# impromptuRong/hd_yolo

Measured on AMD Instinct MI355X. Metric: tiles/sec (640x640) fwd+bwd, higher is better.
Workload: dtype bf16; 1 GPU; metayolo yolov5s 8-class nuclei, 640x640 RGB tiles, batch 64/GPU, train step = fwd + DetLoss + bwd + all-reduce + SGD(nesterov); global_batch=64, parallelism=dp1, world_size=1, backend=none, hw_queues=4

## Files before the change

hd_yolo_amd/build.py:

```python
import os
import subprocess
import sys
from concurrent.futures import ThreadPoolExecutor

HERE = os.path.dirname(os.path.abspath(__file__))
CSRC = os.path.join(HERE, 'csrc')
OUT = os.path.join(CSRC, 'build')
LIB = os.path.join(OUT, 'libhdyolo_hip.so')
SOURCES = ['api.hip', 'conv_dispatch.hip', 'conv_igemm.hip', 'conv3x3.hip', 'conv3x3_c128.hip', 'conv3x3s2.hip', 'conv_deep.hip', 'conv_stem.hip', 'conv_wgrad.hip', 'conv_wgrad3x3.hip', 'conv_wgrad_deep.hip', 'conv_dgrad_s2.hip', 'conv1x1_bwd.hip', 'bn_act.hip', 'pool.hip', 'detect.hip', 'nms_grid.hip', 'slide.hip', 'augment.hip', 'augment_masks.hip', 'score.hip', 'paste.hip', 'mask_score.hip', 'loss.hip', 'roi.hip', 'seg.hip', 'optim.hip', 'exec.hip']
FLAGS = ['--offload-arch=gfx950', '-O3', '-fPIC', '-std=c++17', '-ffp-contract=off', '-Wall', '-Wno-unused-function',
         '-I' + CSRC, '-I' + os.path.join(os.path.dirname(HERE), 'include')]


def _newer(a, bs):
    return os.path.exists(a) and all(os.path.getmtime(a) >= os.path.getmtime(b) for b in bs)


def build(force=False, verbose=True):
    os.makedirs(OUT, exist_ok=True)
    headers = [os.path.join(CSRC, h) for h in os.listdir(CSRC) if h.endswith('.h')]
    headers.append(os.path.join(os.path.dirname(HERE), 'include', 'hdyolo.h'))
    hipcc = os.environ.get('HIPCC', '/opt/rocm/bin/hipcc')

    def compile_one(src):
        s = os.path.join(CSRC, src)
        o = os.path.join(OUT, src.replace('.hip', '.o'))
        if not force and _newer(o, [s] + headers):
            return o
        cmd = [hipcc] + FLAGS + ['-c', s, '-o', o]
        if verbose:
            print(' '.join(cmd), flush=True)
        subprocess.check_call(cmd)
        return o

    with ThreadPoolExecutor(max_workers=min(6, os.cpu_count() or 1)) as ex:
        objs = list(ex.map(compile_one, SOURCES))
    if force or not _newer(LIB, objs):
        cmd = [hipcc, '--offload-arch=gfx950', '-shared', '-fPIC', '-o', LIB] + objs
        if verbose:
            print(' '.join(cmd), flush=True)
        subprocess.check_call(cmd)
    return LIB


if __name__ == '__main__':
    print(build(force='--force' in sys.argv))
```

hd_yolo_amd/csrc/api.hip:

```cpp
#include <stdarg.h>
#include <stdio.h>
#include <stdlib.h>
#include <string.h>

#include <atomic>

#include "common.h"
#include "hdyolo_internal.h"
#include "hdyolo.h"

int hdy_pack_weight_launch(const hdy_pack_desc& d, hipStream_t st);
int hdy_pack_batch_launch(const hdy_pack_desc* table, int n, int total_blocks, hipStream_t st);

static thread_local char g_err[512] = "";

void hdy_set_error(const char* fmt, ...) {
    va_list ap;
    va_start(ap, fmt);
    vsnprintf(g_err, sizeof(g_err), fmt, ap);
    va_end(ap);
}

namespace {
struct OptDef { const char* name; int def; bool flag; };
const OptDef g_opt_def[HDY_OPT_COUNT] = {
    {"HDY_NO_CLASS_WALK", 0, true}, {"HDY_NO_CONV3X3", 0, true}, {"HDY_C3_GRID", 0, false}, {"HDY_NO_CONV3X3S2", 0, false},
    {"HDY_NO_DGRAD_S2", 0, false}, {"HDY_TILE_INTERLEAVE", 1, false}, {"HDY_NO_BIG_TILES", 0, true}, {"HDY_NO_STEM_KERNEL", 0, true},
    {"HDY_WGRAD_BLOCKS", 512, false}, {"HDY_NO_STEM_WGRAD", 0, true}, {"HDY_NO_WGRAD3X3", 0, true}, 
    {"HDY_LOSS_GRID", 2048, false}, {"HDY_NO_DEEP", 0, true}, {"HDY_NO_WGRAD_DEEP", 0, true}, {"HDY_DEEP_BN", 0, false}, {"HDY_DEEP_DEBUG", 0, false}, {"HDY_DEEP_ALL", 1, false}, {"HDY_DEEP_MIN_TILES", 160, false}, {"HDY_DEEP_WALK", 2, false}, {"HDY_NO_BN_REDUCE4", 0, true},
    {"HDY_WGRAD_TILE", 0, false}, {"HDY_SPPF_NO_KEYS", 0, true}, {"HDY_WGRAD_DEEP_KMIN", 192, false}, {"HDY_NO_CONV3X3_C128", 0, true}, {"HDY_NO_F1X1_96", 0, true},
    {"HDY_AP_CHUNK", 0, false}, {"HDY_AP_NO_PRUNE", 0, true},
};
std::atomic<int> g_opt[HDY_OPT_COUNT];
std::once_flag g_opt_once;
void opt_init() {
    std::call_once(g_opt_once, [] {
        for (int i = 0; i < HDY_OPT_COUNT; ++i) {
            const char* v = getenv(g_opt_def[i].name);
            g_opt[i].store(v ? (g_opt_def[i].flag ? 1 : atoi(v)) : g_opt_def[i].def, std::memory_order_relaxed);
        }
    });
}
int opt_index(const char* name) {
    for (int i = 0; name && i < HDY_OPT_COUNT; ++i)
        if (!strcmp(name, g_opt_def[i].name)) return i;
    return -1;
}
thread_local char g_disp_last[64] = "";
std::mutex g_disp_mu;
char g_disp_log[32768] = "";
size_t g_disp_len = 0;
thread_local char g_disp_copy[32768] = "";
}

int hdy_opt(int id) {
    opt_init();
    return g_opt[id].load(std::memory_order_relaxed);
}

void hdy_note_dispatch(const char* what) {
    snprintf(g_disp_last, sizeof(g_disp_last), "%s", what);
    const size_t n = strlen(g_disp_last);
    std::lock_guard<std::mutex> lock(g_disp_mu);
    if (g_disp_len + n + 2 < sizeof(g_disp_log)) {
        memcpy(g_disp_log + g_disp_len, g_disp_last, n);
        g_disp_log[g_disp_len + n] = ';';
        g_disp_log[g_disp_len + n + 1] = 0;
        g_disp_len += n + 1;
    }
}

namespace {

enum { KIND_FWD = 0, KIND_DGRAD = 1, KIND_STEM = 2 };

inline int velems(int dtype) { return dtype == HDY_BF16 ? 8 : 4; }
inline int bke(int dtype) { return 8 * velems(dtype); }
inline size_t esize(int dtype) { return dtype == HDY_BF16 ? 2 : 4; }

inline size_t block_elems(int rows, int kd, int dtype) {
    const int bn = hdy_conv_bn_tile(rows);
    return (size_t)round_up(rows, bn) * round_up(kd, bke(dtype));
}

}

extern "C" {

const char* hdy_last_error(void) { return g_err; }

const char* hdy_last_dispatch(void) { return g_disp_last; }

const char* hdy_dispatch_log(void) {
    std::lock_guard<std::mutex> lock(g_disp_mu);
    memcpy(g_disp_copy, g_disp_log, g_disp_len + 1);
    return g_disp_copy;
}

void hdy_dispatch_log_reset(void) {
    std::lock_guard<std::mutex> lock(g_disp_mu);
    g_disp_log[0] = 0;
    g_disp_len = 0;
    g_disp_last[0] = 0;
}

int hdy_set_option(const char* name, int value) {
    const int i = opt_index(name);
    HDY_ARG(i >= 0, "set_option: unknown option %s", name ? name : "(null)");
    opt_init();
    return g_opt[i].exchange(value, std::memory_order_relaxed);
}
// ... 101 lines not shown
```

hd_yolo_amd/csrc/common.h:

```cpp
#pragma once
#include <hip/hip_runtime.h>
#include <stdint.h>
#include <stddef.h>

#include <mutex>

#define HDY_OK 0
#define HDY_EINVAL (-1)
#define HDY_EUNSUPPORTED (-2)

enum { HDY_F32 = 0, HDY_BF16 = 1 };

void hdy_set_error(const char* fmt, ...);

enum HdyOption {
    HDY_OPT_NO_CLASS_WALK,
    HDY_OPT_NO_CONV3X3,
    HDY_OPT_C3_GRID,
    HDY_OPT_NO_CONV3X3S2,
    HDY_OPT_NO_DGRAD_S2,
    HDY_OPT_TILE_INTERLEAVE,
    HDY_OPT_NO_BIG_TILES,
    HDY_OPT_NO_STEM_KERNEL,
    HDY_OPT_WGRAD_BLOCKS,
    HDY_OPT_NO_STEM_WGRAD,
    HDY_OPT_NO_WGRAD3X3,
    HDY_OPT_LOSS_GRID,
    HDY_OPT_NO_DEEP,
    HDY_OPT_NO_WGRAD_DEEP,
    HDY_OPT_DEEP_BN,
    HDY_OPT_DEEP_DEBUG,
    HDY_OPT_DEEP_ALL,
    HDY_OPT_DEEP_MIN_TILES,
    HDY_OPT_DEEP_WALK,
    HDY_OPT_NO_BN_REDUCE4,
    HDY_OPT_WGRAD_TILE,
    HDY_OPT_SPPF_NO_KEYS,
    HDY_OPT_WGRAD_DEEP_KMIN,
    HDY_OPT_NO_CONV3X3_C128,
    HDY_OPT_NO_F1X1_96,
    HDY_OPT_AP_CHUNK,
    HDY_OPT_AP_NO_PRUNE,
    HDY_OPT_COUNT
};
int hdy_opt(int id);

void hdy_note_dispatch(const char* what);

#define HDY_ARG(cond, ...)                 \
    do {                                   \
        if (!(cond)) {                     \
            hdy_set_error(__VA_ARGS__);    \
            return HDY_EINVAL;             \
        }                                  \
    } while (0)

#define HDY_LAUNCH_CHECK(what)                                                       \
    do {                                                                             \
        hipError_t e__ = hipGetLastError();                                          \
        if (e__ != hipSuccess) {                                                     \
            hdy_set_error("%s: launch failed: %s", what, hipGetErrorString(e__));    \
            return (int)e__;                                                         \
        }                                                                            \
    } while (0)

typedef __bf16 bf16_t;
typedef int i32x4 __attribute__((ext_vector_type(4)));
typedef float f32x4 __attribute__((ext_vector_type(4)));
typedef __bf16 bf16x8 __attribute__((ext_vector_type(8)));
typedef __bf16 bf16x4 __attribute__((ext_vector_type(4)));

#if defined(__HIPCC__)
__device__ __forceinline__ float row_sum16(float v) {
#ifdef HDY_ROW_SUM_SHFL
    for (int m = 1; m < 16; m <<= 1) v += __shfl_xor(v, m);
    return v;
#endif
    v += __builtin_bit_cast(float, __builtin_amdgcn_update_dpp(0, __builtin_bit_cast(int, v), 0x128, 0xF, 0xF, true));
    v += __builtin_bit_cast(float, __builtin_amdgcn_update_dpp(0, __builtin_bit_cast(int, v), 0x124, 0xF, 0xF, true));
    v += __builtin_bit_cast(float, __builtin_amdgcn_update_dpp(0, __builtin_bit_cast(int, v), 0x122, 0xF, 0xF, true));
    v += __builtin_bit_cast(float, __builtin_amdgcn_update_dpp(0, __builtin_bit_cast(int, v), 0x121, 0xF, 0xF, true));
    return v;
}
#endif

struct PerDeviceOnce {
    std::once_flag flag[16];
    template <typename F> void run(F&& fn) {
        int dev = 0;
        (void)hipGetDevice(&dev);
        std::call_once(flag[dev & 15], fn);
    }
};

static inline int cdiv(long long a, long long b) { return (int)((a + b - 1) / b); }
static inline int round_up(int a, int b) { return (a + b - 1) / b * b; }

#ifdef __HIPCC__
union V16 {
    i32x4 i;
    f32x4 f;
    bf16x8 h;
};

__device__ __forceinline__ float silu_f(float u) { return u / (1.0f + __expf(-u)); }
__device__ __forceinline__ float sigmoid_f(float u) { return 1.0f / (1.0f + __expf(-u)); }

template <typename T> __device__ __forceinline__ float to_f32(T v);
template <> __device__ __forceinline__ float to_f32<float>(float v) { return v; }
// ... 97 lines not shown
```

hd_yolo_amd/csrc/conv_dispatch.hip:

```cpp
#include "common.h"
#include "hdyolo_internal.h"
#include "hdyolo.h"

static inline int bke(int dtype) { return dtype == HDY_BF16 ? 64 : 32; }

static ConvPlan conv_fwd_plan(const ConvShape& s, int first = CONV_STEM) {
    ConvPlan p = {};
    if (first <= CONV_STEM && hdy_conv_stem_plan(s, &p)) return p;
    if (first <= CONV_3X3_C64 && hdy_conv3x3_c64_plan(s, &p)) return p;
    if (first <= CONV_3X3_C128 && hdy_conv3x3_c128_plan(s, &p)) return p;
    if (first <= CONV_3X3S2 && hdy_conv3x3s2_plan(s, &p)) return p;
    if (first <= CONV_DGRAD_S2 && hdy_dgrad3x3s2_plan(s, &p)) return p;
    if (first <= CONV_DEEP && hdy_conv_deep_plan(s, &p)) return p;
    hdy_conv_igemm_plan(s, &p);
    return p;
}

extern "C" int hdy_conv_stat_slabs(int N, int H, int W, int C, int K, int R, int S, int stride, int pad, int dtype) {
    const int stem = C == 3 && R == 6 && S == 6 && stride == 2 && pad == 2;
    return conv_fwd_plan(conv_shape(N, H, W, C, K, R, S, stride, pad, dtype, stem, 1)).slabs;
}

static int launch_planned(const ConvArgs& a, const ConvPlan& p, int dtype, int out_f32, hipStream_t st) {
    switch (p.family) {
// ... 118 lines not shown
                c.c_nkb[i] = Kdp / bke(dtype); c.c_oh[i] = ca; c.c_ow[i] = cb; c.c_w[i] = (long long)off;
                off += (size_t)rows_total * Kdp;
            }
        c.w = w_packed_dgrad;
        c.dh0 = c.c_dh[0]; c.dw0 = c.c_dw[0]; c.TH = c.c_TH[0]; c.TW = c.c_TW[0]; c.oh_off = c.ow_off = 0;
        c.Kdp = c.c_nkb[0] * bke(dtype);
        return hdy_conv_launch(c, dgrad_shape(N, H, W, C, K, R, S, stride, pad, dtype), 0, (hipStream_t)stream);
    }
    for (int ca = 0; ca < 2; ++ca)
        for (int cb = 0; cb < 2; ++cb) {
            const Axis ah = class_axis(R, pad, ca), aw = class_axis(S, pad, cb);
            ConvArgs c = a;
            c.Ho = (H - ca + 1) / 2; c.Wo = (W - cb + 1) / 2;
            c.oh_mul = c.ow_mul = 2; c.oh_off = ca; c.ow_off = cb; c.dense_out = 0;
            if (!ah.taps || !aw.taps) {
                HDY_ARG(false, "conv_dgrad: kernel %dx%d pad %d leaves a parity class without taps (unsupported)", R, S, pad);
            }
            if (c.Ho <= 0 || c.Wo <= 0) continue;
            c.dh0 = ah.d0; c.dw0 = aw.d0; c.TH = ah.taps; c.TW = aw.taps;
            c.Kdp = round_up(ah.taps * aw.taps * K, bke(dtype));
            c.w = (const char*)w_packed_dgrad + off * (dtype == HDY_BF16 ? 2 : 4);
            off += (size_t)rows_total * c.Kdp;
            const ConvShape s = {N, Ho, Wo, c.Ho, c.Wo, K, C, ah.taps, aw.taps, 1, -1, 0, dtype, 0, 0, 1};
            const int rc = hdy_conv_launch(c, s, 0, (hipStream_t)stream);
            if (rc) return rc;
        }
    return HDY_OK;
}

extern "C" {

int hdy_conv_fwd(const void* x, int ldx, const void* w_packed, const float* scale, const float* shift, const void* res, int ldr, void* y,
                 int ldy, float* stats, int stat_slabs, int N, int H, int W, int C, int K, int R, int S, int stride, int pad, int act, int accumulate,
                 int dtype, int out_f32, int stem, void* stream) {
    HDY_ARG(!stats || stat_slabs > 0, "conv_fwd: stats given with stat_slabs = %d", stat_slabs);
    HDY_ARG(stride >= 1 && R >= 1 && S >= 1 && pad >= 0, "conv_fwd: bad window");
    HDY_ARG(dtype == HDY_BF16 || dtype == HDY_F32, "conv_fwd: unknown dtype %d", dtype);
    ConvArgs a = {};
    a.x = x; a.w = w_packed; a.y = y; a.scale = scale; a.shift = shift; a.stats = stats; a.stat_cap = stat_slabs; a.res = res; a.ldr = ldr;
    HDY_ARG(!res || ldr >= K, "conv_fwd: residual pitch %d < K", ldr);
    a.N = N;
    a.Ho = conv_out_dim(H, R, stride, pad);
    a.Wo = conv_out_dim(W, S, stride, pad);
    HDY_ARG(a.Ho > 0 && a.Wo > 0, "conv_fwd: empty output");
    a.K = K; a.ldy = ldy;
    a.Hout = a.Ho; a.Wout = a.Wo; a.oh_mul = a.ow_mul = 1; a.oh_off = a.ow_off = 0; a.dense_out = 1;
    a.act = act; a.accumulate = accumulate;
    if (stem) {
        HDY_ARG(C == 3 && R == 6 && S == 6 && stride == 2 && pad == 2 && ldx == 4, "conv_fwd: stem expects C=3 k=6 s=2 p=2 on a 4-channel padded image");
        a.Hin = H + 2 * pad; a.Win = W + 2 * pad; a.C = 24; a.ldx = 4; a.span_pixels = 1;
        a.ih_mul = 2; a.iw_mul = 2; a.dh0 = 0; a.dw0 = 0; a.TH = 6; a.TW = 1;
        a.Kdp = round_up(6 * 24, bke(dtype));
    } else {
        a.Hin = H; a.Win = W; a.C = C; a.ldx = ldx;
        a.ih_mul = stride; a.iw_mul = stride; a.dh0 = -pad; a.dw0 = -pad; a.TH = R; a.TW = S;
        a.Kdp = round_up(R * S * C, bke(dtype));
    }
    return hdy_conv_launch(a, conv_shape(N, H, W, C, K, R, S, stride, pad, dtype, stem != 0, stats != nullptr), out_f32, (hipStream_t)stream);
}

int hdy_conv_dgrad(const void* dy, int lddy, const void* w_packed_dgrad, void* dx, int lddx, int N, int H, int W, int C, int K, int R,
                   int S, int stride, int pad, int accumulate, int dtype, void* stream) {
    return dgrad_impl(dy, lddy, w_packed_dgrad, dx, lddx, N, H, W, C, K, R, S, stride, pad, accumulate, dtype, nullptr, 0, stream);
}

int hdy_conv_dgrad_stats(const void* dy, int lddy, const void* w_packed_dgrad, void* dx, int lddx, int N, int H, int W, int C, int K, int R,
                         int S, int stride, int pad, int accumulate, int dtype, const hdy_stat_req* stats, int nstat, void* stream) {
    HDY_ARG(nstat >= 0 && nstat <= 2 && (nstat == 0 || stats), "conv_dgrad_stats: bad request count");
    HDY_ARG(nstat == 0 || hdy_conv_dgrad_stat_slabs(N, H, W, C, K, R, S, stride, pad, dtype) > 0, "conv_dgrad_stats: this shape cannot serve statistics");
    return dgrad_impl(dy, lddy, w_packed_dgrad, dx, lddx, N, H, W, C, K, R, S, stride, pad, accumulate, dtype, stats, nstat, stream);
}

int hdy_conv_dgrad_stat_slabs(int N, int H, int W, int C, int K, int R, int S, int stride, int pad, int dtype) {
    if (dtype != HDY_BF16 || C % 8 || hdy_conv_bn_tile(C) > 64 || (stride != 1 && stride != 2)) return 0;
    if (stride == 2 && !dgrad_class_walk(H, W, R, S, pad)) return 0;
    return conv_fwd_plan(dgrad_shape(N, H, W, C, K, R, S, stride, pad, dtype), CONV_IGEMM).grid;
}

}

static WgradPlan wgrad_plan(const WgradShape& s, int first = WGRAD_STEM) {
    WgradPlan p = {};
    if (first <= WGRAD_STEM && hdy_wgrad_stem_plan(s, &p)) return p;
    if (first <= WGRAD_3X3 && hdy_wgrad3x3_plan(s, &p)) return p;
    if (first <= WGRAD_DEEP && hdy_wgrad_deep_plan(s, &p)) return p;
    hdy_wgrad_generic_plan(s, &p);
    return p;
}

static int wgrad_launch_planned(const WgradArgs& a, const WgradPlan& p, hipStream_t st) {
    switch (p.family) {
        case WGRAD_STEM: return hdy_wgrad_stem_launch(a, p, st);
        case WGRAD_3X3: return hdy_wgrad3x3_launch(a, p, st);
        case WGRAD_DEEP: return hdy_wgrad_deep_launch(a, p, st);
        default: return hdy_wgrad_generic_launch(a, p, st);
    }
}

static WgradArgs wgrad_args(const WgradShape& s, const void* x, int ldx, const void* dy, int lddy, void* workspace) {
    WgradArgs a = {};
    a.x = x; a.dy = dy; a.partial = (float*)workspace;
    a.N = s.N; a.K = s.K; a.lddy = lddy; a.Ho = s.Ho; a.Wo = s.Wo;
    if (s.stem) {
        a.Hin = s.H + 2 * s.pad; a.Win = s.W + 2 * s.pad; a.C = 24; a.ldx = 4; a.span_pixels = 1;
        a.ih_mul = a.iw_mul = 2; a.dh0 = a.dw0 = 0; a.TH = 6; a.TW = 1;
    } else {
        a.Hin = s.H; a.Win = s.W; a.C = s.C; a.ldx = ldx;
        a.ih_mul = a.iw_mul = s.stride; a.dh0 = a.dw0 = -s.pad; a.TH = s.R; a.TW = s.S;
    }
    return a;
}

static int wgrad_run(const WgradShape& s, const WgradArgs& a, float* grad_a, int K_a, float* grad_b, int K_b, int accumulate, size_t ws_bytes, hipStream_t st) {
    const int VE = s.dtype == HDY_BF16 ? 8 : 4;
    HDY_ARG(grad_a && K_a > 0 && K_a + K_b <= a.K && K_b >= 0 && (K_b == 0) == (grad_b == nullptr), "wgrad: bad gradient split");
    HDY_ARG(a.x && a.dy && a.partial, "wgrad: null pointer");
    HDY_ARG(a.C % VE == 0 && a.K % VE == 0, "wgrad: C=%d and K=%d must be multiples of %d", a.C, a.K, VE);
    HDY_ARG(a.ldx % (a.span_pixels ? 4 : VE) == 0 && a.lddy % VE == 0 && (a.span_pixels || a.ldx >= a.C) && a.lddy >= a.K, "wgrad: bad pitches ldx=%d lddy=%d", a.ldx, a.lddy);
    HDY_ARG(((uintptr_t)a.x & 15) == 0 && ((uintptr_t)a.dy & 15) == 0, "wgrad: x/dy must be 16-byte aligned");
    HDY_ARG((long long)a.N * a.Hin * a.Win < (1LL << 31) && (long long)a.N * a.Ho * a.Wo < (1LL << 31), "wgrad: too many pixels");
    HDY_ARG(ws_bytes >= hdy_conv_wgrad_workspace_bytes(s.N, s.H, s.W, s.C, s.K, s.R, s.S, s.stride, s.pad, s.dtype, s.stem), "wgrad: workspace too small");
    WgradPlan p;
    int rc;
    for (int first = WGRAD_STEM;; first = p.family + 1) {
        p = wgrad_plan(s, first);
        rc = wgrad_launch_planned(a, p, st);
        if (rc != HDY_CONV_DECLINE) break;
    }
    if (rc) return rc;
    return hdy_wgrad_reduce(a.partial, p.splits, s.K, wgrad_cols(s), s.stem, s.C, s.R, s.S, grad_a, K_a, grad_b, K_b, accumulate, st);
}

extern "C" {

size_t hdy_conv_wgrad_workspace_bytes(int N, int H, int W, int C, int K, int R, int S, int stride, int pad, int dtype, int stem) {
    const WgradShape s = wgrad_shape(N, H, W, C, K, R, S, stride, pad, dtype, stem);
    int splits = 0;
    for (int first = WGRAD_STEM; first <= WGRAD_GENERIC;) {
        const WgradPlan p = wgrad_plan(s, first);
        if (p.splits > splits) splits = p.splits;
        first = p.family + 1;
    }
    return (size_t)splits * K * wgrad_cols(s) * sizeof(float);
}

int hdy_conv_wgrad(const void* x, int ldx, const void* dy, int lddy, int N, int H, int W, int C, int K, int R, int S, int stride, int pad,
                   float* grad_a, int K_a, float* grad_b, int K_b, int accumulate, void* workspace, size_t ws_bytes, int dtype, int stem,
                   void* stream) {
    HDY_ARG(dtype == HDY_BF16 || dtype == HDY_F32, "conv_wgrad: unknown dtype %d", dtype);
    const WgradShape s = wgrad_shape(N, H, W, C, K, R, S, stride, pad, dtype, stem != 0);
    HDY_ARG(s.Ho > 0 && s.Wo > 0, "conv_wgrad: empty dy");
    HDY_ARG(!stem || (C == 3 && R == 6 && S == 6 && stride == 2 && pad == 2 && ldx == 4), "conv_wgrad: stem expects C=3 k=6 s=2 p=2 on a 4-channel padded image");
    return wgrad_run(s, wgrad_args(s, x, ldx, dy, lddy, workspace), grad_a, K_a, grad_b, K_b, accumulate, ws_bytes, (hipStream_t)stream);
}

int hdy_conv_wgrad_stem_fused_ok(int N, int H, int W, int K) {
    WgradPlan p;
    return (K == 16 || K == 32 || K == 64) && hdy_wgrad_stem_plan(wgrad_shape(N, H, W, 3, K, 6, 6, 2, 2, HDY_BF16, 1), &p);
}

int hdy_conv_wgrad_stem_fused(const void* x, const void* dz, int lddz, const void* y, int ldy, const float* scale, const float* shift, const float* mean,
                              const float* invstd, const float* c1, const float* c2, int N, int H, int W, int K, float* grad_a, int K_a, float* grad_b,
                              int K_b, int accumulate, void* workspace, size_t ws_bytes, void* stream) {
    HDY_ARG(y, "conv_wgrad_stem_fused: null pointer");
    HDY_ARG(hdy_conv_wgrad_stem_fused_ok(N, H, W, K), "conv_wgrad_stem_fused: shape not served (K in {16, 32, 64}, output a multiple of 16 x 32)");
    const WgradShape s = wgrad_shape(N, H, W, 3, K, 6, 6, 2, 2, HDY_BF16, 1);
    WgradArgs a = wgrad_args(s, x, 4, dz, lddz, workspace);
    a.y = y; a.ldy = ldy; a.bn_scale = scale; a.bn_shift = shift; a.bn_mean = mean; a.bn_invstd = invstd; a.bn_c1 = c1; a.bn_c2 = c2;
    return wgrad_run(s, a, grad_a, K_a, grad_b, K_b, accumulate, ws_bytes, (hipStream_t)stream);
}

}
```

hd_yolo_amd/csrc/hdyolo_internal.h:

```cpp
#pragma once
#include <type_traits>

#include "common.h"

struct StatReq {
    const void* y; int ldy;
    const float *scale, *shift;
    float* slabs;
    int c0, c1, act;
    int nslabs;
};

struct ConvArgs {
    const void* x;
    const void* w;
    void* y;
    const float* scale;
    const float* shift;
    float* stats;
    int stat_cap;
    const void* res;
    int ldr;
    int N, Hin, Win, C, ldx;
    int Ho, Wo, K, ldy;
// ... 60 lines not shown

bool hdy_conv_stem_plan(const ConvShape& s, ConvPlan* p);
bool hdy_conv3x3_c64_plan(const ConvShape& s, ConvPlan* p);
bool hdy_conv3x3_c128_plan(const ConvShape& s, ConvPlan* p);
bool hdy_conv3x3s2_plan(const ConvShape& s, ConvPlan* p);
bool hdy_dgrad3x3s2_plan(const ConvShape& s, ConvPlan* p);
bool hdy_conv_deep_plan(const ConvShape& s, ConvPlan* p);
bool hdy_conv_igemm_plan(const ConvShape& s, ConvPlan* p);

enum { HDY_CONV_DECLINE = -100 };
int hdy_conv_stem_launch(const ConvArgs& a, const ConvPlan& p, int out_f32, hipStream_t st);
int hdy_conv3x3_c64_launch(const ConvArgs& a, const ConvPlan& p, int out_f32, hipStream_t st);
int hdy_conv3x3_c128_launch(const ConvArgs& a, const ConvPlan& p, int out_f32, hipStream_t st);
int hdy_conv3x3s2_launch(const ConvArgs& a, const ConvPlan& p, int out_f32, hipStream_t st);
int hdy_dgrad3x3s2_launch(const ConvArgs& a, const ConvPlan& p, int out_f32, hipStream_t st);
int hdy_conv_deep_launch(const ConvArgs& a, const ConvPlan& p, int out_f32, hipStream_t st);
int hdy_conv_igemm_launch(const ConvArgs& a, const ConvPlan& p, int dtype, int out_f32, hipStream_t st);

inline int hdy_conv_take(const ConvArgs& a, const ConvPlan& p, bool fits, const char* who) {
    if (!fits && !a.stats) return HDY_CONV_DECLINE;
    HDY_ARG(fits, "%s: statistics requested, but this call does not fit the kernel their slabs were sized for (bf16 output, 16-byte aligned x/y/res rows; "
            "ldx=%d ldy=%d)", who, a.ldx, a.ldy);
    HDY_ARG(!a.stats || a.stat_cap == p.slabs, "%s: the statistics array holds %d slabs, this launch writes %d (a kernel-selection option changed between "
            "hdy_conv_stat_slabs and the launch?)", who, a.stat_cap, p.slabs);
    return HDY_OK;
}

inline bool rows_aligned(const ConvArgs& a, bool need_w) {
    return a.ldx % 8 == 0 && a.ldy % 8 == 0 && (((uintptr_t)a.x | (uintptr_t)a.y) & 15) == 0 && (!need_w || (((uintptr_t)a.w & 15) == 0 && a.Kdp % 8 == 0)) &&
           (!a.res || (a.ldr % 8 == 0 && ((uintptr_t)a.res & 15) == 0));
}

inline int epilogue_of(const ConvArgs& a) { return a.act == 1 ? 2 : ((a.scale || a.shift) ? 1 : 0); }

template <typename F> inline void with_stats_epi(bool stats, int epi, F&& f) {
    auto with_epi = [&](auto s) {
        if (epi == 2) f(s, std::integral_constant<int, 2>{});
        else if (epi == 1) f(s, std::integral_constant<int, 1>{});
        else f(s, std::integral_constant<int, 0>{});
    };
    if (stats) with_epi(std::true_type{});
    else with_epi(std::false_type{});
}

inline int hdy_launch_status(const char* who) {
    HDY_LAUNCH_CHECK(who);
    return HDY_OK;
}

inline void hdy_magic(unsigned d, unsigned* mg, int* sh) {
    int s = 0;
    while ((1ull << s) < d) ++s;
    *mg = (unsigned)((((unsigned long long)1 << (31 + s)) + d - 1) / d);
    *sh = s;
}

struct WgradArgs {
    const void* x;
    const void* dy;
    float* partial;
    int N, Hin, Win, C, ldx;
    int Ho, Wo, K, lddy;
    int ih_mul, iw_mul, dh0, dw0, TH, TW;
    int Q, P;
    int splits, pix_per_split;
    int ktiles, qtiles;
    int span_pixels;
    const void* y; int ldy;
    const float *bn_scale, *bn_shift, *bn_mean, *bn_invstd, *bn_c1, *bn_c2;
};

struct WgradShape {
    int N, H, W;
    int Ho, Wo;
    int C, K, R, S, stride, pad, dtype;
    int stem;
};
inline WgradShape wgrad_shape(int N, int H, int W, int C, int K, int R, int S, int stride, int pad, int dtype, int stem) {
    return WgradShape{N, H, W, conv_out_dim(H, R, stride, pad), conv_out_dim(W, S, stride, pad), C, K, R, S, stride, pad, dtype, stem};
}
inline long long wgrad_pixels(const WgradShape& s) { return (long long)s.N * s.Ho * s.Wo; }
inline int wgrad_cols(const WgradShape& s) { return s.R * s.S * (s.stem ? 4 : s.C); }

enum WgradFamily { WGRAD_STEM, WGRAD_3X3, WGRAD_DEEP, WGRAD_GENERIC };

struct WgradPlan {
    int family;
    int variant;
    int grid;
    int splits;
    int pix_per_split;
    int ktiles, qtiles;
    int TOH, TOW, tiles_h, tiles_w;
};

bool hdy_wgrad_stem_plan(const WgradShape& s, WgradPlan* p);
bool hdy_wgrad3x3_plan(const WgradShape& s, WgradPlan* p);
bool hdy_wgrad_deep_plan(const WgradShape& s, WgradPlan* p);
bool hdy_wgrad_generic_plan(const WgradShape& s, WgradPlan* p);

int hdy_wgrad_stem_launch(const WgradArgs& a, const WgradPlan& p, hipStream_t st);
int hdy_wgrad3x3_launch(const WgradArgs& a, const WgradPlan& p, hipStream_t st);
int hdy_wgrad_deep_launch(const WgradArgs& a, const WgradPlan& p, hipStream_t st);
int hdy_wgrad_generic_launch(const WgradArgs& a, const WgradPlan& p, hipStream_t st);
int hdy_wgrad_reduce(const float* partial, int splits, int K, int Q, int mode, int C, int R, int S, float* grad_a, int K_a, float* grad_b, int K_b,
                     int accumulate, hipStream_t st);
```

Measured before the change: 5510 tiles/s.

## Add dedicated 3x3 stride-2 weight-gradient kernel with parity-plane patch tiling

Adds a new wgrad kernel for 3x3 stride-2 pad-1 bf16 convolutions (C=32/K=64 or C,K multiples of 64 with K<192). It stages dy tiles and a parity-split input patch into double-buffered LDS via global_load_lds, and reuses each patch load across three kernel-column taps with MFMA accumulation. The goal is to replace the generic wgrad path for the downsampling convs in the yolov5s backbone. It uses about 140KB of LDS and 768-thread blocks, and it is limited to at most 2 K×C blocks unless an option allows more.

```diff
diff --git a/hd_yolo_amd/build.py b/hd_yolo_amd/build.py
--- a/hd_yolo_amd/build.py
+++ b/hd_yolo_amd/build.py
@@ -7,7 +7,7 @@
 CSRC = os.path.join(HERE, 'csrc')
 OUT = os.path.join(CSRC, 'build')
 LIB = os.path.join(OUT, 'libhdyolo_hip.so')
-SOURCES = ['api.hip', 'conv_dispatch.hip', 'conv_igemm.hip', 'conv3x3.hip', 'conv3x3_c128.hip', 'conv3x3s2.hip', 'conv_deep.hip', 'conv_stem.hip', 'conv_wgrad.hip', 'conv_wgrad3x3.hip', 'conv_wgrad_deep.hip', 'conv_dgrad_s2.hip', 'conv1x1_bwd.hip', 'bn_act.hip', 'pool.hip', 'detect.hip', 'nms_grid.hip', 'slide.hip', 'augment.hip', 'augment_masks.hip', 'score.hip', 'paste.hip', 'mask_score.hip', 'loss.hip', 'roi.hip', 'seg.hip', 'optim.hip', 'exec.hip']
+SOURCES = ['api.hip', 'conv_dispatch.hip', 'conv_igemm.hip', 'conv3x3.hip', 'conv3x3_c128.hip', 'conv3x3s2.hip', 'conv_deep.hip', 'conv_stem.hip', 'conv_wgrad.hip', 'conv_wgrad3x3.hip', 'conv_wgrad3x3s2.hip', 'conv_wgrad_deep.hip', 'conv_dgrad_s2.hip', 'conv1x1_bwd.hip', 'bn_act.hip', 'pool.hip', 'detect.hip', 'nms_grid.hip', 'slide.hip', 'augment.hip', 'augment_masks.hip', 'score.hip', 'paste.hip', 'mask_score.hip', 'loss.hip', 'roi.hip', 'seg.hip', 'optim.hip', 'exec.hip']
 FLAGS = ['--offload-arch=gfx950', '-O3', '-fPIC', '-std=c++17', '-ffp-contract=off', '-Wall', '-Wno-unused-function',
          '-I' + CSRC, '-I' + os.path.join(os.path.dirname(HERE), 'include')]
 
diff --git a/hd_yolo_amd/csrc/api.hip b/hd_yolo_amd/csrc/api.hip
--- a/hd_yolo_amd/csrc/api.hip
+++ b/hd_yolo_amd/csrc/api.hip
@@ -26,7 +26,7 @@
 const OptDef g_opt_def[HDY_OPT_COUNT] = {
     {"HDY_NO_CLASS_WALK", 0, true}, {"HDY_NO_CONV3X3", 0, true}, {"HDY_C3_GRID", 0, false}, {"HDY_NO_CONV3X3S2", 0, false},
     {"HDY_NO_DGRAD_S2", 0, false}, {"HDY_TILE_INTERLEAVE", 1, false}, {"HDY_NO_BIG_TILES", 0, true}, {"HDY_NO_STEM_KERNEL", 0, true},
-    {"HDY_WGRAD_BLOCKS", 512, false}, {"HDY_NO_STEM_WGRAD", 0, true}, {"HDY_NO_WGRAD3X3", 0, true}, 
+    {"HDY_WGRAD_BLOCKS", 512, false}, {"HDY_NO_STEM_WGRAD", 0, true}, {"HDY_NO_WGRAD3X3", 0, true}, {"HDY_NO_WGRAD3X3S2", 0, false},
     {"HDY_LOSS_GRID", 2048, false}, {"HDY_NO_DEEP", 0, true}, {"HDY_NO_WGRAD_DEEP", 0, true}, {"HDY_DEEP_BN", 0, false}, {"HDY_DEEP_DEBUG", 0, false}, {"HDY_DEEP_ALL", 1, false}, {"HDY_DEEP_MIN_TILES", 160, false}, {"HDY_DEEP_WALK", 2, false}, {"HDY_NO_BN_REDUCE4", 0, true},
     {"HDY_WGRAD_TILE", 0, false}, {"HDY_SPPF_NO_KEYS", 0, true}, {"HDY_WGRAD_DEEP_KMIN", 192, false}, {"HDY_NO_CONV3X3_C128", 0, true}, {"HDY_NO_F1X1_96", 0, true},
     {"HDY_AP_CHUNK", 0, false}, {"HDY_AP_NO_PRUNE", 0, true},
diff --git a/hd_yolo_amd/csrc/common.h b/hd_yolo_amd/csrc/common.h
--- a/hd_yolo_amd/csrc/common.h
+++ b/hd_yolo_amd/csrc/common.h
@@ -25,6 +25,7 @@
     HDY_OPT_WGRAD_BLOCKS,
     HDY_OPT_NO_STEM_WGRAD,
     HDY_OPT_NO_WGRAD3X3,
+    HDY_OPT_NO_WGRAD3X3S2,
     HDY_OPT_LOSS_GRID,
     HDY_OPT_NO_DEEP,
     HDY_OPT_NO_WGRAD_DEEP,
diff --git a/hd_yolo_amd/csrc/conv_dispatch.hip b/hd_yolo_amd/csrc/conv_dispatch.hip
--- a/hd_yolo_amd/csrc/conv_dispatch.hip
+++ b/hd_yolo_amd/csrc/conv_dispatch.hip
@@ -224,6 +224,7 @@
 static WgradPlan wgrad_plan(const WgradShape& s, int first = WGRAD_STEM) {
     WgradPlan p = {};
     if (first <= WGRAD_STEM && hdy_wgrad_stem_plan(s, &p)) return p;
+    if (first <= WGRAD_3X3S2 && hdy_wgrad3x3s2_plan(s, &p)) return p;
     if (first <= WGRAD_3X3 && hdy_wgrad3x3_plan(s, &p)) return p;
     if (first <= WGRAD_DEEP && hdy_wgrad_deep_plan(s, &p)) return p;
     hdy_wgrad_generic_plan(s, &p);
@@ -233,6 +234,7 @@
 static int wgrad_launch_planned(const WgradArgs& a, const WgradPlan& p, hipStream_t st) {
     switch (p.family) {
         case WGRAD_STEM: return hdy_wgrad_stem_launch(a, p, st);
+        case WGRAD_3X3S2: return hdy_wgrad3x3s2_launch(a, p, st);
         case WGRAD_3X3: return hdy_wgrad3x3_launch(a, p, st);
         case WGRAD_DEEP: return hdy_wgrad_deep_launch(a, p, st);
         default: return hdy_wgrad_generic_launch(a, p, st);
diff --git a/hd_yolo_amd/csrc/conv_wgrad3x3s2.hip b/hd_yolo_amd/csrc/conv_wgrad3x3s2.hip
--- /dev/null
+++ b/hd_yolo_amd/csrc/conv_wgrad3x3s2.hip
@@ -0,0 +1,305 @@
+#include <stdlib.h>
+
+#include "common.h"
+#include "hdyolo_internal.h"
+#include "hdyolo.h"
+
+__device__ uint4 g_hdy_zero16_w3s2[4];
+
+namespace {
+
+struct W3S2Args {
+    const void* x; int ldx;
+    const void* dy; int lddy;
+    float* partial;
+    int N, Ho, Wo, C, K, Hin, Win;
+    int TOH, tiles_h, tiles_w;
+    int nkb, ncb, nsplit;
+};
+
+constexpr int W3S2_KB = 64;
+constexpr int W3S2_TOW = 16;
+
+template <int CB> struct W3S2Cfg {
+    static constexpr int RB = CB * 2;
+    static constexpr int CPR = RB / 16;
+    static constexpr int MAXTOH = CB == 32 ? 10 : 6;
+    static constexpr int ROWS_I = 1024 / RB;
+    static constexpr int MAXTP = MAXTOH * W3S2_TOW;
+    static constexpr int MAXPP = ((2 * MAXTOH + 1) * (2 * W3S2_TOW + 1) + ROWS_I - 1) / ROWS_I * ROWS_I;
+    static constexpr int DY_I = MAXTP / 8;
+    static constexpr int P_I = MAXPP / ROWS_I;
+    static constexpr int DY_Q = DY_I / 4;
+    static constexpr int P_Q = (P_I + 7) / 8;
+    static constexpr int NQ = DY_Q > P_Q ? DY_Q : P_Q;
+    static constexpr int DYB = MAXTP * W3S2_KB * 2;
+    static constexpr int BUF = DYB + MAXPP * RB;
+    static constexpr int NSTEP = MAXTP / 32;
+    static constexpr int LDS = 2 * BUF;
+    static_assert(MAXTP % 32 == 0 && MAXPP % ROWS_I == 0 && DY_I % 4 == 0, "whole MFMA steps, whole DMA instructions");
+    static_assert(MAXPP * RB < 65536, "patch offsets are kept in 16 bits");
+    static_assert(LDS <= 140 * 1024, "LDS headroom for the other stream");
+};
+
+template <int CB> __device__ __forceinline__ int psw(int row) {
+    if constexpr (CB == 64) return fsw3(row);
+    else return (((row >> 1) ^ (row >> 3)) & 1) << 1;
+}
+
+__device__ __forceinline__ int plane_base(int rp, int cp, int TOH, int TOW) {
+    const int n00 = (TOH + 1) * (TOW + 1), n01 = (TOH + 1) * TOW, n10 = TOH * (TOW + 1);
+    return rp ? (cp ? n00 + n01 + n10 : n00 + n01) : (cp ? n00 : 0);
+}
+
+template <int CB>
+__global__ __launch_bounds__(768) void wgrad3x3s2_kernel(const W3S2Args p) {
+    using Cfg = W3S2Cfg<CB>;
+    constexpr int KB = W3S2_KB;
+    constexpr int MTW = KB / 32, NTW = CB / 32;
+    extern __shared__ __attribute__((aligned(16))) unsigned char smem[];
+
+    const int tid = threadIdx.x, lane = tid & 63, wave = __builtin_amdgcn_readfirstlane(tid >> 6);
+    const int tr = wave >> 2, wm = (wave >> 1) & 1, wn = wave & 1;
+    const int g = lane >> 4, i16 = lane & 15, q4 = i16 >> 2, p4 = i16 & 3;
+    const int blocks = p.nkb * p.ncb;
+    const int bid = xcd_remap(blockIdx.x, gridDim.x);
+    const int split = bid / blocks, blk = bid - split * blocks;
+    const int kb = blk / p.ncb, cb = blk - kb * p.ncb;
+    constexpr int TOW = W3S2_TOW;
+    const int TOH = p.TOH;
+    const int TP = TOH * TOW, PP = (2 * TOH + 1) * (2 * TOW + 1);
+    const int steps = (TP + 31) / 32;
+    const bf16_t* __restrict__ x = (const bf16_t*)p.x;
+    const bf16_t* __restrict__ dy = (const bf16_t*)p.dy;
+    const unsigned char* zero = (const unsigned char*)g_hdy_zero16_w3s2;
+    const int per_img = p.tiles_h * p.tiles_w;
+    const int tiles = p.N * per_img;
+    const bool dy_loader = wave < 4;
+
+    int l_off[Cfg::NQ], l_yx[Cfg::NQ];
+#pragma unroll
+    for (int i = 0; i < Cfg::NQ; ++i) {
+        l_off[i] = 0;
+        l_yx[i] = 0x7FFF7FFF;
+        if (dy_loader && i < Cfg::DY_Q) {
+            const int row = (wave + 4 * i) * 8 + (lane >> 3);
+            const int ty = row / TOW, tx = row - ty * TOW;
+            const int lc = (lane & 7) ^ fsw3(row);
+            l_off[i] = (ty * p.Wo + tx) * p.lddy + kb * KB + lc * 8;
+            if (row < TP) l_yx[i] = (ty << 16) | tx;
+        } else if (!dy_loader && i < Cfg::P_Q) {
+            const int row = (wave - 4 + 8 * i) * Cfg::ROWS_I + lane / Cfg::CPR;
+            const int lc = (lane % Cfg::CPR) ^ psw<CB>(row);
+            if (row < PP) {
+                const int b01 = plane_base(0, 1, TOH, TOW), b10 = plane_base(1, 0, TOH, TOW), b11 = plane_base(1, 1, TOH, TOW);
+                const int rp = row >= b10, cp = rp ? row >= b11 : row >= b01;
+                const int rel = row - plane_base(rp, cp, TOH, TOW), pw = TOW + 1 - cp;
+                const int yy = rel / pw, xx = rel - yy * pw;
+                const int py = 2 * yy + rp, px = 2 * xx + cp;
+                l_off[i] = ((py - 1) * p.Win + (px - 1)) * p.ldx + cb * CB + lc * 8;
+                l_yx[i] = (py << 16) | px;
+            }
+        }
+    }
+    auto issue = [&](int t, int buf) {
+        unsigned char* sD = smem + buf * Cfg::BUF;
+        unsigned char* sP = sD + Cfg::DYB;
+        const int n = t / per_img, rem = t - n * per_img;
+        const int th = rem / p.tiles_w, tw = rem - th * p.tiles_w;
+        const int oh0 = th * TOH, ow0 = tw * TOW;
+        if (dy_loader) {
+            const bf16_t* org = dy + ((size_t)(n * p.Ho + oh0) * p.Wo + ow0) * p.lddy;
+            const int hy = p.Ho - oh0, hx = p.Wo - ow0;
+#pragma unroll
+            for (int i = 0; i < Cfg::DY_Q; ++i) {
+                const int d = wave + 4 * i;
+                if (d * 8 >= steps * 32) continue;
+                const bool ok = ((l_yx[i] >> 16) < hy) & ((l_yx[i] & 0xFFFF) < hx);
+                const void* src = ok ? (const void*)(org + l_off[i]) : (const void*)zero;
+                __builtin_amdgcn_global_load_lds((const void __attribute__((address_space(1)))*)src,
+                                                 (void __attribute__((address_space(3)))*)(sD + d * 1024), 16, 0, 0);
+            }
+        } else {
+            const int ih0 = 2 * oh0 - 1, iw0 = 2 * ow0 - 1;
+            const bf16_t* org = x + ((size_t)(n * p.Hin + 2 * oh0) * p.Win + 2 * ow0) * p.ldx;
+#pragma unroll
+            for (int i = 0; i < Cfg::P_Q; ++i) {
+                const int e = wave - 4 + 8 * i;
+                if (e >= Cfg::P_I || e * Cfg::ROWS_I >= PP) continue;
+                const int py = l_yx[i] >> 16, px = l_yx[i] & 0xFFFF;
+                const bool ok = ((unsigned)(ih0 + py) < (unsigned)p.Hin) & ((unsigned)(iw0 + px) < (unsigned)p.Win) & (py < 0x7FFF);
+                const void* src = ok ? (const void*)(org + l_off[i]) : (const void*)zero;
+                __builtin_amdgcn_global_load_lds((const void __attribute__((address_space(1)))*)src,
+                                                 (void __attribute__((address_space(3)))*)(sP + e * 1024), 16, 0, 0);
+            }
+        }
+    };
+
+    constexpr int NSTEP = Cfg::NSTEP;
+    unsigned ptab[NSTEP][3];
+    int dtab[2];
+    {
+        const int lcb = (wn * (CB / 2)) >> 3, lca = (wm * (KB / 2)) >> 3;
+#pragma unroll
+        for (int s = 0; s < NSTEP; ++s)
+#pragma unroll
+            for (int sx = 0; sx < 3; ++sx) ptab[s][sx] = 0;
+#pragma unroll
+        for (int s = 0; s < NSTEP; ++s)
+#pragma unroll
+            for (int h = 0; h < 2; ++h) {
+                const int ra = s * 32 + 8 * g + q4 + 4 * h;
+                int ty = ra / TOW, tx = ra - ty * TOW;
+                if (ra >= TP) ty = tx = 0;
+#pragma unroll
+                for (int sx = 0; sx < 3; ++sx) {
+                    const int cp = sx & 1;
+                    const int pr = plane_base(tr & 1, cp, TOH, TOW) + (ty + (tr >> 1)) * (TOW + 1 - cp) + tx + (sx >> 1);
+                    ptab[s][sx] |= (unsigned)(pr * Cfg::RB + (((lcb + (p4 >> 1)) ^ psw<CB>(pr)) << 4) + (p4 & 1) * 8) << (16 * h);
+                }
+                if (s == 0) dtab[h] = ra * 128 + (((lca + (p4 >> 1)) ^ fsw3(ra)) << 4) + (p4 & 1) * 8;
+            }
+    }
+
+    f32x4 acc[3][MTW][NTW];
+#pragma unroll
+    for (int t = 0; t < 3; ++t)
+#pragma unroll
+        for (int a = 0; a < MTW; ++a)
+#pragma unroll
+            for (int b = 0; b < NTW; ++b) acc[t][a][b] = f32x4{0.f, 0.f, 0.f, 0.f};
+
+    typedef int i32x2 __attribute__((ext_vector_type(2)));
+#define W3S2_TRR(dst, addr) asm volatile("ds_read_b64_tr_b16 %0, %1" : "=v"(dst) : "v"(addr) : "memory")
+#define W3S2_LGKM(n) do { asm volatile("s_waitcnt lgkmcnt(%0)" ::"n"(n) : "memory"); __builtin_amdgcn_sched_barrier(0); } while (0)
+    const unsigned lds0 = (unsigned)(uintptr_t)(const __attribute__((address_space(3))) unsigned char*)smem;
+    if (split < tiles) issue(split, 0);
+    int cur = 0;
+    for (int t = split; t < tiles; t += p.nsplit, cur ^= 1) {
+        asm volatile("s_waitcnt vmcnt(0)" ::: "memory");
+        __builtin_amdgcn_s_barrier();
+        asm volatile("" ::: "memory");
+        if (t + p.nsplit < tiles) issue(t + p.nsplit, cur ^ 1);
+        const unsigned sD = lds0 + cur * Cfg::BUF;
+        const unsigned sP = sD + Cfg::DYB;
+#pragma unroll
+        for (int s = 0; s < NSTEP; ++s) {
+            if (s < steps) {
+                i32x2 al[MTW], ah[MTW], bl[2][NTW], bh[2][NTW];
+#pragma unroll
+                for (int a = 0; a < MTW; ++a) {
+                    W3S2_TRR(al[a], sD + s * 4096 + (dtab[0] ^ (a << 5)));
+                    W3S2_TRR(ah[a], sD + s * 4096 + (dtab[1] ^ (a << 5)));
+                }
+                {
+                    unsigned pk = ptab[s][0];
+                    asm volatile("" : "+v"(pk));
+#pragma unroll
+                    for (int b = 0; b < NTW; ++b) {
+                        W3S2_TRR(bl[0][b], sP + ((pk & 0xFFFFu) ^ (b << 5)));
+                        W3S2_TRR(bh[0][b], sP + ((pk >> 16) ^ (b << 5)));
+                    }
+                }
+#pragma unroll
+                for (int sx = 0; sx < 3; ++sx) {
+                    if (sx < 2) {
+                        unsigned pk = ptab[s][sx + 1];
+                        asm volatile("" : "+v"(pk));
+#pragma unroll
+                        for (int b = 0; b < NTW; ++b) {
+                            W3S2_TRR(bl[(sx + 1) & 1][b], sP + ((pk & 0xFFFFu) ^ (b << 5)));
+                            W3S2_TRR(bh[(sx + 1) & 1][b], sP + ((pk >> 16) ^ (b << 5)));
+                        }
+                        W3S2_LGKM(2 * NTW);
+                    } else {
+                        W3S2_LGKM(0);
+                    }
+                    V16 af[MTW], bf[NTW];
+#pragma unroll
+                    for (int a = 0; a < MTW; ++a) af[a].i = i32x4{al[a][0], al[a][1], ah[a][0], ah[a][1]};
+#pragma unroll
+                    for (int b = 0; b < NTW; ++b) bf[b].i = i32x4{bl[sx & 1][b][0], bl[sx & 1][b][1], bh[sx & 1][b][0], bh[sx & 1][b][1]};
+#pragma unroll
+                    for (int a = 0; a < MTW; ++a)
+#pragma unroll
+                        for (int b = 0; b < NTW; ++b)
+                            acc[sx][a][b] = __builtin_amdgcn_mfma_f32_16x16x32_bf16(af[a].h, bf[b].h, acc[sx][a][b], 0, 0, 0);
+                }
+            }
+        }
+    }
+#undef W3S2_TRR
+#undef W3S2_LGKM
+
+    const int Q = 9 * p.C;
+    float* out = p.partial + (size_t)split * p.K * Q;
+#pragma unroll
+    for (int sx = 0; sx < 3; ++sx)
+#pragma unroll
+        for (int a = 0; a < MTW; ++a)
+#pragma unroll
+            for (int rr = 0; rr < 4; ++rr) {
+                const int k = kb * KB + wm * (KB / 2) + a * 16 + g * 4 + rr;
+#pragma unroll
+                for (int b = 0; b < NTW; ++b)
+                    out[(size_t)k * Q + (tr * 3 + sx) * p.C + cb * CB + wn * (CB / 2) + b * 16 + i16] = acc[sx][a][b][rr];
+            }
+}
+
+}
+
+bool hdy_wgrad3x3s2_plan(const WgradShape& s, WgradPlan* pl) {
+    const int C = s.C, K = s.K, Ho = s.Ho;
+    const int opt = hdy_opt(HDY_OPT_NO_WGRAD3X3S2);
+    if (s.stem || s.R != 3 || s.S != 3 || s.pad != 1 || s.stride != 2 || s.dtype != HDY_BF16 || opt == 1) return false;
+    int CB;
+    if (C == 32 && K == 64) CB = 32;
+    else if (C % 64 == 0 && K % 64 == 0 && K < 192) CB = 64;
+    else return false;
+    *pl = WgradPlan{};
+    pl->family = WGRAD_3X3S2;
+    pl->variant = CB == 64;
+    pl->ktiles = K / W3S2_KB;
+    pl->qtiles = C / CB;
+    const int blocks = pl->ktiles * pl->qtiles;
+    if (blocks > 4 || (blocks > 2 && opt != 2)) return false;
+    const int maxtp = CB == 32 ? W3S2Cfg<32>::MAXTP : W3S2Cfg<64>::MAXTP, maxpp = CB == 32 ? W3S2Cfg<32>::MAXPP : W3S2Cfg<64>::MAXPP;
+    pl->TOW = W3S2_TOW;
+    pl->TOH = maxtp / pl->TOW;
+    if (pl->TOH > Ho) pl->TOH = Ho;
+    if (pl->TOH < 1) return false;
+    pl->tiles_h = cdiv(Ho, pl->TOH);
+    pl->TOH = cdiv(Ho, pl->tiles_h);
+    if ((2 * pl->TOH + 1) * (2 * pl->TOW + 1) > maxpp || pl->TOH * pl->TOW > maxtp) return false;
+    pl->tiles_w = cdiv(s.Wo, pl->TOW);
+    const long long tiles = (long long)s.N * pl->tiles_h * pl->tiles_w;
+    WgradPlan gen;
+    hdy_wgrad_generic_plan(s, &gen);
+    long long ns = 256 / blocks;
+    if (ns > gen.splits) ns = gen.splits;
+    if (ns > tiles) ns = tiles;
+    if (ns < 1) ns = 1;
+    pl->splits = (int)ns;
+    pl->grid = blocks * pl->splits;
+    return true;
+}
+
+template <int CB> static void w3s2_start(const W3S2Args& a, int grid, hipStream_t st) {
+    constexpr int lds = W3S2Cfg<CB>::LDS;
+    static PerDeviceOnce attr_once;
+    attr_once.run([&] { (void)hipFuncSetAttribute((const void*)wgrad3x3s2_kernel<CB>, hipFuncAttributeMaxDynamicSharedMemorySize, lds); });
+    hipLaunchKernelGGL((wgrad3x3s2_kernel<CB>), dim3(grid), dim3(768), lds, st, a);
+}
+
+int hdy_wgrad3x3s2_launch(const WgradArgs& w, const WgradPlan& pl, hipStream_t st) {
+    if (w.ldx % 8 || w.lddy % 8 || (((uintptr_t)w.x | (uintptr_t)w.dy) & 15)) return HDY_CONV_DECLINE;
+    W3S2Args a = {};
+    a.x = w.x; a.ldx = w.ldx; a.dy = w.dy; a.lddy = w.lddy; a.partial = w.partial;
+    a.N = w.N; a.Ho = w.Ho; a.Wo = w.Wo; a.C = w.C; a.K = w.K; a.Hin = w.Hin; a.Win = w.Win;
+    a.TOH = pl.TOH; a.tiles_h = pl.tiles_h; a.tiles_w = pl.tiles_w;
+    a.nkb = pl.ktiles; a.ncb = pl.qtiles; a.nsplit = pl.splits;
+    hdy_note_dispatch("wgrad3x3s2");
+    if (pl.variant) w3s2_start<64>(a, pl.grid, st);
+    else w3s2_start<32>(a, pl.grid, st);
+    return hdy_launch_status("wgrad3x3s2");
+}
diff --git a/hd_yolo_amd/csrc/hdyolo_internal.h b/hd_yolo_amd/csrc/hdyolo_internal.h
--- a/hd_yolo_amd/csrc/hdyolo_internal.h
+++ b/hd_yolo_amd/csrc/hdyolo_internal.h
@@ -166,7 +166,7 @@
 inline long long wgrad_pixels(const WgradShape& s) { return (long long)s.N * s.Ho * s.Wo; }
 inline int wgrad_cols(const WgradShape& s) { return s.R * s.S * (s.stem ? 4 : s.C); }
 
-enum WgradFamily { WGRAD_STEM, WGRAD_3X3, WGRAD_DEEP, WGRAD_GENERIC };
+enum WgradFamily { WGRAD_STEM, WGRAD_3X3S2, WGRAD_3X3, WGRAD_DEEP, WGRAD_GENERIC };
 
 struct WgradPlan {
     int family;
@@ -179,11 +179,13 @@
 };
 
 bool hdy_wgrad_stem_plan(const WgradShape& s, WgradPlan* p);
+bool hdy_wgrad3x3s2_plan(const WgradShape& s, WgradPlan* p);
 bool hdy_wgrad3x3_plan(const WgradShape& s, WgradPlan* p);
 bool hdy_wgrad_deep_plan(const WgradShape& s, WgradPlan* p);
 bool hdy_wgrad_generic_plan(const WgradShape& s, WgradPlan* p);
 
 int hdy_wgrad_stem_launch(const WgradArgs& a, const WgradPlan& p, hipStream_t st);
+int hdy_wgrad3x3s2_launch(const WgradArgs& a, const WgradPlan& p, hipStream_t st);
 int hdy_wgrad3x3_launch(const WgradArgs& a, const WgradPlan& p, hipStream_t st);
 int hdy_wgrad_deep_launch(const WgradArgs& a, const WgradPlan& p, hipStream_t st);
 int hdy_wgrad_generic_launch(const WgradArgs& a, const WgradPlan& p, hipStream_t st);
```

New measurement: 5520 tiles/s, median of 3. No clear change (+0.2%).
